# Bitlab-UMA/IMSAME

Measured on AMD Instinct MI355X. Metric: reads aligned/sec (node), 1M×150bp vs 50Mbp ref, 1/2/4/8 MI355X, higher is better.
Workload: dtype int16

## Files before the change

### imsame_amd/csrc/imsame_dev.hip

```cpp
#include <hip/hip_runtime.h>
#include <stdint.h>
#include <stdio.h>
#include <stdlib.h>
#include <string.h>
#include <math.h>
#include <limits.h>
#include <time.h>
#include <sched.h>
#include <vector>
#include <algorithm>
#include <thread>
#include <mutex>
#include <condition_variable>
#include "../../include/imsame_dev.h"

#include "tables.h"
#include "nw_kernel.hip"
#include "nw16_kernel.hip"
#include "nwl_kernel.hip"
#include "nwp_kernel.hip"
#include "seed_kernel.hip"
#include "round_policy.h"


// ... 255 lines not shown
    uint64_t tab_L = 0;
    uint32_t tab_ymax = 0, tab_xmax = 0;
    DBuf tb, bnd, paths, ck;
    DBuf slotbits;
    int np_part_cu = -1;
    DBuf np_tb, np_ck;
    imsame_ctx *np_owner = nullptr;
    uint64_t paths_cap_dev = 0, paths_n = 0;
    double paths_hint = 0;
    std::vector<uint32_t> paths_host;
    bool paths_on_host = false;
    DBuf rc_in, rc_out, rc_a, rc_b, rc_c;
    uint64_t ev_db_len = 0;
    bool use_wcap = false, use_wstart = false;
    DBuf wcap, wout, wstart;
    std::vector<imsame_ctx *> subs;
    bool is_sub = false, paths_split = false;
    std::vector<uint64_t> lane_paths;
    hipEvent_t origin = nullptr;
    hipEvent_t ev_w = nullptr;
    hipEvent_t ev_wd = nullptr;
    std::vector<std::pair<float, float>> nw_iv;
    struct TlEv { char kind; int round; uint32_t n; float a, b; };
    std::vector<TlEv> tl;
    int cur_round = 0;
    std::mutex iv_mu, persist_mu;
    int nlanes = 1;
    std::vector<uint32_t> part_paths;
    uint32_t stall_us[2] = {0, 0}, stall_n[2] = {0, 0};
};

static inline uint64_t hqs(const imsame_ctx *c, uint64_t r) { return c->hq[r - c->q_lo]; }
#define QB_READS 4096
static uint64_t range_ymax(const imsame_ctx *c, uint64_t a, uint64_t b) {
    uint64_t m = 0;
    auto len = [&](uint64_t r) { return hqs(c, r + 1) - hqs(c, r); };
    uint64_t blk = (a - c->q_lo + QB_READS - 1) / QB_READS, r = c->q_lo + blk * QB_READS;
    for (uint64_t x = a; x < std::min(b, r); ++x) m = std::max(m, len(x));
    for (; r + QB_READS <= b; r += QB_READS, ++blk) m = std::max<uint64_t>(m, c->hqb[blk]);
    for (uint64_t x = std::max(a, r); x < b; ++x) m = std::max(m, len(x));
    return m;
}
static inline const uint8_t *dev_q(const imsame_ctx *c) { return (const uint8_t *)((uintptr_t)c->q.p - c->q_base); }
static inline const uint32_t *dev_qw(const imsame_ctx *c) {
    return (const uint32_t *)((uintptr_t)c->qw.p - c->qw_base * sizeof(uint32_t));
}
static inline const uint64_t *dev_qs(const imsame_ctx *c) {
    return (const uint64_t *)((uintptr_t)c->q_start.p - c->q_lo * sizeof(uint64_t));
}
#define QPAD 64

enum { C_NCAND = 0, C_NCAND2, C_NNEXT, C_NCANDB, C_NCAND2B, C_NNEXT2, C_WORKB,
       C_WORK, C_WORK2, C_PATHS, C_FLAGS, C_ERR, C_HITS, C_CELLS, C_NACC, C_REDO,
       C_PROF, C_WIN = C_PROF + 12, C_FBK, C_SWORK, C_DBG = C_SWORK + 3, C_WASTE = C_DBG + 8,
       C_NSLOTS };

#define STALL_US_MAX 20000u
__global__ void __launch_bounds__(64) stall_kernel(uint32_t ticks) {
    const uint64_t t0 = wall_clock64();
    for (uint32_t i = 0; i < (1u << 20); ++i) {
        if (wall_clock64() - t0 >= ticks) break;
        __builtin_amdgcn_s_sleep(32);
    }
}
static void stall_parse(imsame_ctx *c) {
    c->stall_us[0] = c->stall_us[1] = 0;
    c->stall_n[0] = c->stall_n[1] = 0;
    const char *e = getenv("IMSAME_DEBUG_STALL");
    while (e && *e) {
        const int side = (*e == 'A' || *e == 'a') ? 0 : (*e == 'B' || *e == 'b') ? 1 : -1;
        if (side >= 0 && e[1] == ':') {
            const long us = strtol(e + 2, nullptr, 10);
            c->stall_us[side] = (uint32_t)std::max<long>(0, std::min<long>(us, (long)STALL_US_MAX));
        }
        e = strchr(e, ',');
        if (e) ++e;
    }
}
static int stall(imsame_ctx *c, hipStream_t s) {
    const int side = s == c->stream ? 0 : 1;
    if (!c->stall_us[side]) return 0;
    stall_kernel<<<1, 64, 0, s>>>(c->stall_us[side] * 100u);
    HIPCHK(hipGetLastError());
    __atomic_fetch_add(&c->stall_n[side], 1u, __ATOMIC_RELAXED);
    return 0;
}
#define STALL(c, s) do { if (int src_ = stall((c), (s))) return src_; } while (0)

static double now_ms() {
    struct timespec ts; clock_gettime(CLOCK_MONOTONIC, &ts);
    return ts.tv_sec * 1e3 + ts.tv_nsec * 1e-6;
}

extern "C" void imsame_params_default(imsame_params *p) {
    memset(p, 0, sizeof *p);
    p->min_e = 1 / powl(10, 20);
    p->min_coverage = 0.5; p->min_identity = 0.5;
    p->igap = -5; p->egap = -2;
    p->max_read_size = IMSAME_MAX_READ_SIZE;
    p->want_paths = 0;
}

extern "C" const char *imsame_strerror(int code) {
    switch (code) {
    case IMSAME_OK: return "ok";
    case IMSAME_E_HIP: return "HIP runtime error";
    case IMSAME_E_OOM: return "out of memory";
// ... 1509 lines not shown
                           (uint32_t *)(ctr + cls[k].work), c->db.as<uint8_t>(), c->db_start.as<uint64_t>(), qd, qsd,
                           pcap, &ms, k == 0 ? crow : nullptr);
            if (rc) return rc;
            rec_launch(st, pl, cls[k].n, ms);
            if ((rc = upd_launch(cls[k].cr, cls[k].cs, cls[k].n, cls[k].o, nxt, C_NNEXT, s))) return rc;
        }
        uint64_t nn = 0;
        HIPCHK(hipMemcpyAsync(&nn, ctr + C_NNEXT, 8, hipMemcpyDeviceToHost, s));
        LANE_SYNC(c, s);
        if (getenv("IMSAME_DEBUG_ROUNDS")) {
            std::vector<imsame_read_result> o(std::min<uint32_t>(n1, 6));
            std::vector<uint32_t> cr(o.size());
            if (!o.empty()) {
                HIPCHK(hipMemcpy(o.data(), c->cout.p, o.size() * 64, hipMemcpyDeviceToHost));
                HIPCHK(hipMemcpy(cr.data(), c->cread.p, o.size() * 4, hipMemcpyDeviceToHost));
            }
            uint64_t dg[8], nacc = 0;
            HIPCHK(hipMemcpy(dg, ctr + C_DBG, sizeof dg, hipMemcpyDeviceToHost));
            HIPCHK(hipMemcpy(&nacc, ctr + C_NACC, 8, hipMemcpyDeviceToHost));
            fprintf(stderr, "[round %llu] active=%u spec=%u budget=%u cand=%u+%u next=%llu acc_total=%llu "
                    "outcomes(err0 pause0 done0 err pause exh full)=%llu %llu %llu %llu %llu %llu %llu |",
                    (unsigned long long)st.rounds, nact, S.spec, S.budget, n1, n2, (unsigned long long)nn,
                    (unsigned long long)nacc, (unsigned long long)dg[0], (unsigned long long)dg[1],
                    (unsigned long long)dg[2], (unsigned long long)dg[3], (unsigned long long)dg[4],
                    (unsigned long long)dg[5], (unsigned long long)dg[6]);
            for (size_t k = 0; k < o.size(); ++k)
                fprintf(stderr, " r%u/s%llu st%u len%u id%u y%u", cr[k], (unsigned long long)o[k].db_seq, o[k].status,
                        o[k].length, o[k].identities, o[k].ylen);
            fprintf(stderr, "\n");
        }
        nact = (uint32_t)nn;
        std::swap(act, nxt);
    }
    uint64_t hc[C_NSLOTS];
    HIPCHK(hipMemcpyAsync(hc, ctr, C_NSLOTS * 8, hipMemcpyDeviceToHost, s));
    LANE_SYNC(c, s);
    const double t_d2h = now_ms();
    HIPCHK(hipMemcpyAsync(res, c->res.p, (uint64_t)n * 64, hipMemcpyDeviceToHost, s));
    LANE_SYNC(c, s);
    st.ms_d2h = now_ms() - t_d2h;
    st.n_hits = hc[C_HITS];
    st.seed_windows = hc[C_SWORK]; st.seed_entries = hc[C_SWORK + 1]; st.seed_ext_chunks = hc[C_SWORK + 2];
    st.nw_cells = hc[C_CELLS];
    st.n_accepted = hc[C_NACC];
    st.nw_redo = (uint32_t)hc[C_REDO];
    st.nw_win = (uint32_t)hc[C_WIN];
    st.nw_fallback = (uint32_t)hc[C_FBK];
    st.nw_spec_waste = hc[C_WASTE];
    if (getenv("IMSAME_NW_PROF")) {
        const double tot = (double)(hc[C_PROF] + hc[C_PROF + 1] + hc[C_PROF + 2] + hc[C_PROF + 3] + hc[C_PROF + 4]);
        const double ghz = hc[C_PROF + 5] ? tot / (double)hc[C_PROF + 5] * 0.1 : 0.0;
        fprintf(stderr, "[nwprof] setup %.3f sweep1 %.3f reduce %.3f sweep2 %.3f walk %.3f (fractions of %.4g wave-cycles) "
                "clock_ghz %.3f best_cells(weak: last_row last_col<=40 <=200 higher | predicted: in out) "
                "%llu %llu %llu %llu | %llu %llu\n", hc[C_PROF] / tot, hc[C_PROF + 1] / tot, hc[C_PROF + 2] / tot,
                hc[C_PROF + 3] / tot, hc[C_PROF + 4] / tot, tot, ghz, (unsigned long long)hc[C_PROF + 6],
                (unsigned long long)hc[C_PROF + 7], (unsigned long long)hc[C_PROF + 8], (unsigned long long)hc[C_PROF + 9],
                (unsigned long long)hc[C_PROF + 10], (unsigned long long)hc[C_PROF + 11]);
    }
    if ((c->stall_us[0] || c->stall_us[1]) && getenv("IMSAME_DEBUG_ROUNDS"))
        fprintf(stderr, "[stall] A=%u B=%u\n", c->stall_n[0], c->stall_n[1]);
    st.nw_launch_ms = st.nw_launches ? st.ms_nw / st.nw_launches : 0;
    st.nw_bytes = 2 * st.nw_cells;
    int ret = IMSAME_OK;
    if (hc[C_FLAGS] & 4) return IMSAME_E_HIP;
    if (hc[C_FLAGS] & 8) return IMSAME_E_ARG;
    if (hc[C_ERR] != ~0ull) {
        st.err_read = hc[C_ERR] >> 32; st.err_dbseq = hc[C_ERR] & 0xFFFFFFFFull;
        ret = IMSAME_E_READ_TOO_LONG;
    }
    if (p->want_paths) {
        uint64_t used = std::min<uint64_t>((uint32_t)hc[C_PATHS], pcap);
        if (hc[C_FLAGS] & 1) {
            rc = rewalk_lost(c, p, read_from, n, res, ymax, xcap, ycap, short_y, &used, &st);
            if (rc) return rc;
        }
        c->paths_n = used;
        c->paths_hint = std::min(64.0, (double)used / n);
        if (paths_used) *paths_used = used;
        if (used > paths_cap) { if (ret == IMSAME_OK) ret = IMSAME_E_PATHS; }
        else if (used) {
            HIPCHK(hipMemcpyAsync(paths, c->paths.p, used * 4, hipMemcpyDeviceToHost, s));
            HIPCHK(hipStreamSynchronize(s));
        }
    }
    st.ms_total = now_ms() - t_start;
    if (stats) *stats = st;
    return ret;
}

static void span_ms(const std::vector<std::pair<float, float>> &v, double *first, double *last) {
    *first = *last = 0;
    for (size_t k = 0; k < v.size(); ++k) {
        if (k == 0 || v[k].first < *first) *first = v[k].first;
        if (k == 0 || v[k].second > *last) *last = v[k].second;
    }
}

static double union_ms(std::vector<std::pair<float, float>> v) {
    std::sort(v.begin(), v.end());
    double tot = 0, a = 0, b = -1;
    for (const auto &x : v) {
        if (x.first > b) { if (b > a) tot += b - a; a = x.first; b = x.second; }
        else b = std::max<double>(b, x.second);
    }
    if (b > a) tot += b - a;
    return tot;
}

#define LANE_MIN 32768
#define LANE_READS 40000
// ... 496 lines not shown
```

### imsame_amd/csrc/nw16_kernel.hip

```cpp

#define NW16_K   10
#define NW16_K5  5
#define NW16_K3  3
#define NW16_K3_YMAX 150
#define NW16_BIG 16384
__host__ __device__ constexpr int nw16_ck(int K) { return K <= 3 ? 14 : K <= 5 ? 32 : 48; }
__host__ __device__ constexpr int nw16_nst(int K) { return 4 * K + 5; }
__host__ __device__ constexpr int nw16_nrec(int K) { return K <= 8 ? 2 : K <= 10 ? 3 : 2 * ((K + 7) / 8); }
#define NW16_K19 19
#define NW16_K19_OFF 2
#define NW16_K19_YLEN (8 * NW16_K19 - NW16_K19_OFF)
#define NW16_NOROW INT32_MIN
#define NW16_WIN_UP 32
#define NW16_WIN_DOWN 24
#define NW16_WIN_MAX 448
#define NW16_WIN_BOTTOM 40
#define NW16_BAND2 4

__host__ static inline bool nw16_fits(int64_t ig, int64_t eg, uint64_t xcap, uint64_t ymax, int K = NW16_K) {
    if (ig > 0 || eg > 0 || ymax > (uint64_t)NW_W / 2 || ymax == 0) return false;
    const uint64_t G = (ymax + K - 1) / K, ycols = G * K;
    const uint64_t aig = (uint64_t)(-ig), aeg = (uint64_t)(-eg);
    if (aig > 8191 || aeg > 8191) return false;
    const uint64_t R = 4 * ycols + aig + aeg * (xcap + 64 + ycols + 2) + 16;
    return R <= 8191;
}

WV_DEVICE uint32_t pk1(int v) { return (uint32_t)(uint16_t)v * 0x10001u; }
WV_DEVICE uint32_t pk2(int lo, int hi) { return (uint32_t)(uint16_t)lo | ((uint32_t)(uint16_t)hi << 16); }
WV_DEVICE int pk_half(uint32_t v, int h) { return (int)(int16_t)(h ? (v >> 16) : (v & 0xFFFFu)); }
#define NW16_H 0x80008000u
WV_DEVICE int pk_score(uint32_t v, int h) { return (int)(h ? (v >> 16) : (v & 0xFFFFu)) - 32768; }
WV_DEVICE uint32_t base_code(uint8_t b) { return (b >> 1) & 3u; }

#ifndef NW16_ROWTAB
#define NW16_ROWTAB 1
#endif
#define NW16_TBL_LO 0xFCFCFC04u
#define NW16_TBL_HI 0xFFFFFF00u
#if NW16_ROWTAB
#define NW16_XSH_A 3
#define NW16_XSH_B 5
#else
#define NW16_XSH_A 0
#define NW16_XSH_B 2
#endif
#define NW16_XM_A (3u << NW16_XSH_A)
#define NW16_XM_B (3u << NW16_XSH_B)
struct Nw16Row { uint32_t lo, hi; };
WV_DEVICE Nw16Row nw16_row(uint32_t xb) {
#if NW16_ROWTAB
    return {8u << (xb & 31u), 8u << ((xb >> 2) & 0x18u)};
#else
    return {wv_perm(xb >> 2, xb & 3u, 0x04040000u), 0u};
#endif
}
WV_DEVICE uint32_t nw16_ycol(uint32_t ya, uint32_t yb) {
#if NW16_ROWTAB
    return ya | (0x0Cu << 8) | ((yb + 4u) << 16) | (0x0Cu << 24);
#else
    return ya | ((ya | 4u) << 8) | (yb << 16) | ((yb | 4u) << 24);
#endif
}
WV_DEVICE uint32_t nw16_sc(const Nw16Row &r, uint32_t ycol) {
#if NW16_ROWTAB
    return wv_perm(r.hi, r.lo, ycol);
#else
    return wv_perm(NW16_TBL_HI, NW16_TBL_LO, r.lo ^ ycol);
#endif
// ... 74 lines not shown
};

__host__ __device__ static inline size_t nw16_wave_lds(int GPW, int xstride) {
    return (size_t)GPW * xstride + 64 * 8 * 4;
}

template <int K, bool LAST, bool TWO, int OFF = 0>
__device__ __forceinline__ void nw16_wave(const NwLaunch &P, uint8_t *wsm, const int lane, const uint32_t slot) {
    constexpr int NST = nw16_nst(K), NREC = nw16_nrec(K), CK = nw16_ck(K);
    constexpr uint32_t RECB = 64u * 4u * NREC;
    const int G = P.G, GPW = P.GPW;
    const int g = lane / G, gl = lane - g * G;
    const bool in_group = g < GPW;
    const int gg = in_group ? g : 0;
    int *red = (int *)(wsm + (size_t)GPW * P.xstride);
    uint32_t *tbw = P.tb + (uint64_t)slot * P.tb_wave_dw;
    uint32_t *ckw = TWO ? P.ck + (uint64_t)slot * P.ck_wave_dw + lane : nullptr;
    const int ig = P.igap, eg = P.egap;

    unsigned long long ph[5] = {0, 0, 0, 0, 0}, tq = P.prof ? wv_clock() : 0, rt0 = P.prof ? wv_realtime() : 0;
    auto mark = [&](const int k) {
        if (P.prof) { const unsigned long long n = wv_clock(); ph[k] += n - tq; tq = n; }
    };
    for (uint32_t ntask = 0;; ++ntask) {
        if (P.slot_bits && ntask) break;
        uint32_t base = 0;
        if (lane == 0) base = wv_atomic_add(P.counter, (uint32_t)(2 * GPW));
        base = wv_first(base);
        if (base >= P.n_cand) break;
        bool valid[2];
        uint32_t cidx[2], sid[2] = {0, 0};
        int xl[2] = {0, 0}, yl[2] = {0, 0}, prow[2] = {NW16_NOROW, NW16_NOROW};
        const uint8_t *Yp[2] = {P.q, P.q}, *Xg[2] = {P.db, P.db};
        for (int h = 0; h < 2; ++h) {
            cidx[h] = base + 2 * g + h;
            valid[h] = in_group && cidx[h] < P.n_cand;
        }
        for (int h = 0; h < 2; ++h) {
            const uint32_t w = valid[h] ? cidx[h] : cidx[0];
            if (valid[0]) {
                const uint32_t c = P.perm ? P.perm[w] : w;
                cidx[h] = c;
                if (P.cand_row) prow[h] = P.cand_row[c];
                const uint32_t rd = P.cand_read[c];
                sid[h] = P.cand_sid[c];
                const uint64_t xo = P.db_start[sid[h]];
                xl[h] = (int)(P.db_start[sid[h] + 1] - xo);
                Xg[h] = P.db + xo;
                const uint64_t yo = P.q_start[rd];
                Yp[h] = P.q + yo; yl[h] = (int)(P.q_start[rd + 1] - yo);
            }
        }
        const int xlp = max(xl[0], xl[1]);
        uint8_t *X8 = wsm + (size_t)(valid[0] ? g : 0) * P.xstride;
        if (valid[0]) {
            const int nch = (xlp + 15) >> 4;
            for (int c = gl; c < nch; c += G) {
                const int k0 = c << 4;
                uint32_t w[2][4];
                for (int h = 0; h < 2; ++h) {
                    if (k0 + 16 <= xl[h]) {
                        __builtin_memcpy(w[h], Xg[h] + k0, 16);
                    } else {
#pragma unroll
                        for (int q = 0; q < 4; ++q) {
                            uint32_t v = 0;
#pragma unroll
                            for (int b = 0; b < 4; ++b) v |= (uint32_t)Xg[h][min(k0 + 4 * q + b, xl[h] - 1)] << (8 * b);
                            w[h][q] = v;
                        }
                    }
                }
                uint32_t o[4];
#pragma unroll
                for (int q = 0; q < 4; ++q)
                    o[q] = (((w[0][q] >> 1) << NW16_XSH_A) & (NW16_XM_A * 0x01010101u)) |
                           (((w[1][q] >> 1) << NW16_XSH_B) & (NW16_XM_B * 0x01010101u));
                __builtin_memcpy(X8 + k0, o, 16);
            }
        }
        wv_lds_sync();

        int xmax = valid[0] ? xlp : 0, xmin = valid[0] ? min(xl[0], xl[1]) : INT_MAX;
        for (int o = 32; o > 0; o >>= 1) {
            xmax = max(xmax, wv_shfl_xor(xmax, o));
            xmin = min(xmin, wv_shfl_xor(xmin, o));
        }
        xmax = (int)wv_first((uint32_t)xmax); xmin = (int)wv_first((uint32_t)xmin);
        int tw0 = INT_MAX - 2, tw1 = INT_MAX - 2;
        if (TWO && P.cand_row) {
            int lo = INT_MAX, hi = INT_MIN, none = 0;
            for (int h = 0; h < 2; ++h) {
                if (!valid[h]) continue;
                if (prow[h] == NW16_NOROW) {
                    if (P.win_bottom < 0) { none = 1; continue; }
                    lo = min(lo, xl[h] - 1 - P.win_bottom);
                    hi = max(hi, xl[h] - 1);
                    continue;
                }
                lo = min(lo, prow[h] - P.win_up);
                hi = max(hi, prow[h] + yl[h] - 1 + P.win_down);
            }
            for (int o = 32; o > 0; o >>= 1) {
                lo = min(lo, wv_shfl_xor(lo, o));
                hi = max(hi, wv_shfl_xor(hi, o));
                none = max(none, wv_shfl_xor(none, o));
            }
            if (!none && lo <= hi) {
                int a = max(lo, 1), b = min(hi, xmax) + G;
                a -= (a & 1) ^ 1; b += (b & 1) ^ 1;
                if (b > a && b - a <= NW16_WIN_MAX) { tw0 = a; tw1 = b; }
            }
            tw0 = (int)wv_first((uint32_t)tw0); tw1 = (int)wv_first((uint32_t)tw1);
        }
        const int tb0 = TWO ? tw0 : 0;

        const int j0 = gl * K - OFF;
        const bool leadc0 = gl == 0;
        const int xcl = max(xlp - 1, 0);
        const uint32_t NBIG = pk1(-NW16_BIG) ^ NW16_H, EGN = pk1(-eg), IGEN = pk1(-(ig + eg));
        uint32_t yreg[K], lastm[K];
        bool ownC[2], lact[2];
        for (int h = 0; h < 2; ++h) {
            ownC[h] = valid[0] && yl[h] >= 2 && yl[h] - 1 >= j0 && yl[h] - 1 < j0 + K;
            lact[h] = valid[0] && j0 < yl[h];
        }
#pragma unroll
        for (int s = 0; s < K; ++s) {
            const int j = j0 + s;
            const uint32_t ya = (valid[0] && j >= 0 && j < yl[0]) ? base_code(Yp[0][j]) : 0u;
            const uint32_t yb = (valid[0] && j >= 0 && j < yl[1]) ? base_code(Yp[1][j]) : 0u;
            yreg[s] = nw16_ycol(ya, yb);
            lastm[s] = ((ownC[0] && yl[0] - 1 - j0 == s) ? 0x0000FFFFu : 0u) |
                       ((ownC[1] && yl[1] - 1 - j0 == s) ? 0xFFFF0000u : 0u);
        }
        uint32_t xrow = valid[0] ? X8[0] : 0u;
        const Nw16Row xr0 = nw16_row(xrow);
        uint32_t yprev = nw16_ycol(0u, 0u);
        if (valid[0] && j0 > 0) {
            const uint32_t ya = base_code(Yp[0][min(j0 - 1, yl[0] - 1)]), yb = base_code(Yp[1][min(j0 - 1, yl[1] - 1)]);
            yprev = nw16_ycol(ya, yb);
        }
        const uint32_t t0prev = nw16_sc_biased(nw16_sc(xr0, yprev));
        uint32_t A[K], B[K], dI[K], mcS[K], u0[K];
#pragma unroll
        for (int s = 0; s < K; ++s) {
            A[s] = nw16_sc_biased(nw16_sc(xr0, yreg[s]));
            B[s] = A[s];
        }
#pragma unroll
        for (int s = 0; s < K; ++s) {
            dI[s] = ((s == 0) ? t0prev : A[s - 1]) - IGEN;
            mcS[s] = dI[s];
            u0[s] = dI[s];
            if (j0 + s == 1) mcS[s] = pk1(NW16_BIG) ^ NW16_H;
        }
        uint32_t I1 = t0prev, I2 = t0prev;
        uint32_t outT = A[K - 1], outMS = 0, outL = 0;
        const int tend = xmax - 1 + G;
        xrow = valid[0] ? X8[min(max(1 - gl, 0), xcl)] : 0u;
        uint32_t bestC = pk1(-NW16_BIG) ^ NW16_H, bestCi = 0, ipk = pk1(1 - gl);
        int bestR[2] = {INT_MIN, INT_MIN}, bestRj[2] = {0, 0};
        const uint32_t limp = pk2(xl[0] - 2, xl[1] - 2);
        uint8_t *tb3 = (uint8_t *)tbw;

        auto step = [&](const bool PRE, const bool CAREFUL, const bool TB, const int t, uint32_t (&cur)[K],
                        const uint32_t (&own)[K], uint32_t &in0, const uint32_t in1) {
            const uint32_t sN = (uint32_t)wv_shr1((int)outT), mS = (uint32_t)wv_shr1((int)outMS),
                           mL0 = (uint32_t)wv_shr1((int)outL);
            const int i = t - gl;
            const Nw16Row xr = nw16_row(xrow);
            xrow = CAREFUL ? X8[min(max(i + 1, 0), xcl)] : X8[i + 1];
            const bool pre = PRE && i < 1;
            const bool row1 = CAREFUL && i <= 1;
            uint32_t mfS = mS, l0 = mL0;
            TbWords<K> tw = {};
#pragma unroll
            for (int s = 0; s < K; ++s) {
                const uint32_t d0 = (s == 0) ? in1 : own[s - 1];
                const uint32_t tl = (s == 0) ? sN : cur[s - 1];
                const uint32_t sc = nw16_sc(xr, yreg[s]);
                const uint32_t up = row1 ? NBIG : u0[s];
                const uint32_t lu = pk_maxu(l0, up);
                uint32_t v = nw16_add_sc(pk_maxu(d0, lu), sc);
                if (s == OFF) v = leadc0 ? nw16_sc_biased(sc) : v;
                cur[s] = pre ? own[s] : v;
                const uint32_t P2 = TB ? wv_perm(pk_sub(l0, up), pk_sub(d0, lu), 0x0B0A0908u) : 0u;
                const uint32_t mU = pk_neg_mask(pk_sub(mcS[s], dI[s]));
                const uint32_t u0n = wv_bfi(mU, dI[s], u0[s]) - EGN;
                u0[s] = row1 ? u0[s] : u0n;
                mcS[s] = wv_bfi(mU, dI[s], mcS[s]);
                const uint32_t mnL = pk_neg_mask(pk_sub(tl, mfS));
                dI[s] = d0 - IGEN;
                l0 = wv_bfi(mnL, l0 - EGN, dI[s]);
                mfS = wv_bfi(mnL, mfS, d0);
                if (s == OFF) { mfS = leadc0 ? NBIG : mfS; l0 = leadc0 ? NBIG : l0; }
                if (TB) tw.add(s, P2, mU, mnL);
            }
            if (TB) tw.store((uint32_t *)(tb3 + ((uint32_t)(t - tb0) * RECB + (uint32_t)lane * (4u * NREC))));
            uint32_t vl = cur[LAST ? K - 1 : 0];
            if (!LAST)
#pragma unroll
                for (int s = 1; s < K; ++s) vl = wv_bfi(lastm[s], cur[s], vl);
            uint32_t km = pk_neg_mask(pk_sub(vl, bestC));
            if (CAREFUL) {
                km |= pk_neg_mask(pk_sub(limp, ipk)) | pk_neg_mask(pk_sub(ipk, pk1(1)));
                if (i >= 1 && (i == xl[0] - 1 || i == xl[1] - 1)) {
                    for (int h = 0; h < 2; ++h) {
                        if (!lact[h] || i != xl[h] - 1) continue;
#pragma unroll
                        for (int s = 0; s < K; ++s) {
                            const int j = j0 + s, val = pk_score(cur[s], h);
                            if (j >= 1 && j < yl[h] && val >= bestR[h]) { bestR[h] = val; bestRj[h] = j; }
                        }
                    }
                }
            }
            bestC = wv_bfi(km, bestC, vl);
            bestCi = wv_bfi(km, bestCi, ipk);
            ipk = pk_add(ipk, 0x10001u);
            in0 = pre ? in1 : sN;
            outT = cur[K - 1]; outMS = mfS; outL = l0;
        };
        constexpr bool TB1 = !TWO;
        auto save = [&](const int m) {
            uint32_t *p = ckw + (uint32_t)m * (NST * 64u);
#pragma unroll
            for (int s = 0; s < K; ++s) {
                p[s * 64] = A[s]; p[(K + s) * 64] = B[s];
                p[(2 * K + s) * 64] = mcS[s]; p[(3 * K + s) * 64] = u0[s];
            }
            p[4 * K * 64] = I1; p[(4 * K + 1) * 64] = I2;
            p[(4 * K + 2) * 64] = outT; p[(4 * K + 3) * 64] = outMS; p[(4 * K + 4) * 64] = outL;
        };
        int nextck = 1 + CK, mck = 1;
        auto ck = [&](const int t) { if (TWO && t == nextck) { save(mck); ++mck; nextck += CK; } };
        if (TWO) save(0);
        mark(0);
        auto inwin = [&](const int tt) { return TWO && tt >= tw0 && tt < tw1; };
        int t = 1;
        for (; t + 1 < tend && t <= G + 1; t += 2) {
            ck(t);
            if (inwin(t)) {
                step(true, true, true, t, A, B, I2, I1);
                step(true, true, true, t + 1, B, A, I1, I2);
            } else {
                step(true, true, TB1, t, A, B, I2, I1);
                step(true, true, TB1, t + 1, B, A, I1, I2);
            }
        }
        auto fast = [&](const bool TBW, const int tlim) {
            for (; t + 1 <= tlim; t += 2) {
                ck(t);
                step(false, false, TBW, t, A, B, I2, I1);
                step(false, false, TBW, t + 1, B, A, I1, I2);
            }
        };
        fast(TB1, min(xmin - 2, tw0 - 1));
        if (TWO) {
            fast(true, min(xmin - 2, tw1 - 1));
            fast(false, xmin - 2);
        }
        for (; t + 1 < tend; t += 2) {
            ck(t);
            if (inwin(t)) {
                step(false, true, true, t, A, B, I2, I1);
                step(false, true, true, t + 1, B, A, I1, I2);
            } else {
                step(false, true, TB1, t, A, B, I2, I1);
                step(false, true, TB1, t + 1, B, A, I1, I2);
            }
        }
        if (t < tend) {
            if (inwin(t)) step(true, true, true, t, A, B, I2, I1);
            else          step(true, true, TB1, t, A, B, I2, I1);
        }
        wv_mem_sync();
        mark(1);

        for (int h = 0; h < 2; ++h) {
            red[lane * 8 + 4 * h + 0] = bestR[h];
            red[lane * 8 + 4 * h + 1] = bestRj[h];
            red[lane * 8 + 4 * h + 2] = ownC[h] ? pk_score(bestC, h) : INT_MIN;
            red[lane * 8 + 4 * h + 3] = pk_half(bestCi, h);
        }
        wv_lds_sync();
        int bscore[2], bx[2], by[2];
        for (int h = 0; h < 2; ++h) {
            int bR = INT_MIN, bRj = 0, bC = INT_MIN, bCi = 0;
            if (in_group)
                for (int k = 0; k < G; ++k) {
                    const int *e = red + (g * G + k) * 8 + 4 * h;
                    if (e[0] > bR || (e[0] == bR && e[1] > bRj)) { bR = e[0]; bRj = e[1]; }
                    if (e[2] > bC || (e[2] == bC && e[3] > bCi)) { bC = e[2]; bCi = e[3]; }
                }
            if (bR >= bC) { bscore[h] = bR; bx[h] = xl[h] - 1; by[h] = bRj; }
            else          { bscore[h] = bC; bx[h] = bCi; by[h] = yl[h] - 1; }
        }
        wv_lds_sync();
        if (P.prof && in_group && gl == 0)
            for (int h = 0; h < 2; ++h) {
                if (!valid[h]) continue;
                int b;
                if (prow[h] == NW16_NOROW) {
                    const int up = xl[h] - 1 - bx[h];
                    b = up == 0 ? 6 : up <= 40 ? 7 : up <= 200 ? 8 : 9;
                } else {
                    b = (bx[h] >= prow[h] - P.win_up && bx[h] <= prow[h] + yl[h] - 1 + P.win_down) ? 10 : 11;
                }
                wv_atomic_add64(P.prof + b, 1ull);
            }
        mark(2);
        if (!TWO) {
            for (int h = 0; h < 2; ++h) {
                const TbAcc16<K, OFF> acc16 = {tbw, X8, Yp[h], gg, G, h, 0};
                nw_finish(P, acc16, xl[h], yl[h], valid[h], gg, gl, G, bscore[h], bx[h], by[h], cidx[h], sid[h]);
            }
            wv_lds_sync();
            mark(4);
            continue;
        }

        bool todo[2] = {valid[0], valid[1]};
        if (tw1 > tw0) {
            bool cov[2];
            for (int h = 0; h < 2; ++h) cov[h] = todo[h] && bx[h] + G <= tw1;
            if (wv_any(cov[0] || cov[1])) {
                for (int h = 0; h < 2; ++h) {
                    TbAcc16<K, OFF> acc16 = {tbw, X8, Yp[h], gg, G, h, tw0};
                    acc16.t1 = tw1;
                    const bool lost = nw_finish(P, acc16, xl[h], yl[h], cov[h], gg, gl, G, bscore[h], bx[h], by[h],
                                                cidx[h], sid[h]);
                    if (cov[h]) todo[h] = lost;
                    if (cov[h] && !lost && gl == 0 && in_group && P.win) wv_atomic_add(P.win, 1u);
                }
                wv_mem_sync();
            }
            mark(4);
        }
        int t0h[2] = {1, 1};
        auto step2 = [&](const bool MASK, const int tau, uint32_t (&cur)[K], const uint32_t (&own)[K],
                         uint32_t &in0, const uint32_t in1) {
            const uint32_t sN = (uint32_t)wv_shr1((int)outT), mS = (uint32_t)wv_shr1((int)outMS),
                           mL0 = (uint32_t)wv_shr1((int)outL);
            const int iA = t0h[0] + tau - gl, iB = t0h[1] + tau - gl;
            const Nw16Row xr = nw16_row(xrow);
            xrow = (X8[min(max(iA + 1, 0), xcl)] & NW16_XM_A) | (X8[min(max(iB + 1, 0), xcl)] & NW16_XM_B);
            const uint32_t pm = !MASK ? 0u : (iA < 1 ? 0x0000FFFFu : 0u) | (iB < 1 ? 0xFFFF0000u : 0u);
            const uint32_t r1 = !MASK ? 0u : (iA <= 1 ? 0x0000FFFFu : 0u) | (iB <= 1 ? 0xFFFF0000u : 0u);
            uint32_t mfS = mS, l0 = mL0;
            TbWords<K> tw = {};
#pragma unroll
            for (int s = 0; s < K; ++s) {
                const uint32_t d0 = (s == 0) ? in1 : own[s - 1];
                const uint32_t tl = (s == 0) ? sN : cur[s - 1];
                const uint32_t sc = nw16_sc(xr, yreg[s]);
                const uint32_t up = MASK ? wv_bfi(r1, NBIG, u0[s]) : u0[s];
                const uint32_t lu = pk_maxu(l0, up);
                uint32_t v = nw16_add_sc(pk_maxu(d0, lu), sc);
                if (s == OFF) v = leadc0 ? nw16_sc_biased(sc) : v;
                cur[s] = MASK ? wv_bfi(pm, own[s], v) : v;
                const uint32_t P2 = wv_perm(pk_sub(l0, up), pk_sub(d0, lu), 0x0B0A0908u);
                const uint32_t mU = pk_neg_mask(pk_sub(mcS[s], dI[s]));
                const uint32_t u0n = wv_bfi(mU, dI[s], u0[s]) - EGN;
                u0[s] = MASK ? wv_bfi(r1, u0[s], u0n) : u0n;
                mcS[s] = wv_bfi(mU, dI[s], mcS[s]);
                const uint32_t mnL = pk_neg_mask(pk_sub(tl, mfS));
                dI[s] = d0 - IGEN;
                l0 = wv_bfi(mnL, l0 - EGN, dI[s]);
                mfS = wv_bfi(mnL, mfS, d0);
                if (s == OFF) { mfS = leadc0 ? NBIG : mfS; l0 = leadc0 ? NBIG : l0; }
                tw.add(s, P2, mU, mnL);
            }
            tw.store((uint32_t *)(tb3 + ((uint32_t)tau * RECB + (uint32_t)lane * (4u * NREC))));
            in0 = MASK ? wv_bfi(pm, in1, sN) : sN;
            outT = cur[K - 1]; outMS = mfS; outL = l0;
        };
        for (int att = wv_any(todo[0] || todo[1]) ? 0 : 3; att < 3; ++att) {
            int n2 = 0;
            for (int h = 0; h < 2; ++h) {
                const int lo = bx[h] - (att == 0 ? P.band_w : NW16_BAND2 * P.band_w) - 1;
                t0h[h] = (att < 2 && lo >= 0) ? 1 + CK * (lo / CK) : 1;
                if (todo[h]) n2 = max(n2, bx[h] + G - t0h[h]);
            }
            for (int o = 32; o > 0; o >>= 1) n2 = max(n2, wv_shfl_xor(n2, o));
            {
                const uint32_t *pa = ckw + (uint32_t)((t0h[0] - 1) / CK) * (NST * 64u);
                const uint32_t *pb = ckw + (uint32_t)((t0h[1] - 1) / CK) * (NST * 64u);
                auto ld = [&](const int r) { return wv_bfi(0x0000FFFFu, pa[r * 64], pb[r * 64]); };
#pragma unroll
                for (int s = 0; s < K; ++s) {
                    A[s] = ld(s); B[s] = ld(K + s);
                    mcS[s] = ld(2 * K + s); u0[s] = ld(3 * K + s);
                }
                I1 = ld(4 * K); I2 = ld(4 * K + 1);
                outT = ld(4 * K + 2); outMS = ld(4 * K + 3); outL = ld(4 * K + 4);
#pragma unroll
                for (int s = 0; s < K; ++s) dI[s] = (s ? A[s - 1] : I2) - IGEN;
                xrow = (X8[min(max(t0h[0] - gl, 0), xcl)] & NW16_XM_A) | (X8[min(max(t0h[1] - gl, 0), xcl)] & NW16_XM_B);
            }
            int tmin = min(t0h[0], t0h[1]);
            for (int o = 32; o > 0; o >>= 1) tmin = min(tmin, wv_shfl_xor(tmin, o));
            const int tau_m = G + 1 - tmin;
            int tau = 0;
            for (; tau + 1 < n2 && tau < tau_m; tau += 2) {
                step2(true, tau, A, B, I2, I1);
                step2(true, tau + 1, B, A, I1, I2);
            }
            for (; tau + 1 < n2; tau += 2) {
                step2(false, tau, A, B, I2, I1);
                step2(false, tau + 1, B, A, I1, I2);
            }
            if (tau < n2) step2(true, tau, A, B, I2, I1);
            wv_mem_sync();
            mark(3);
            for (int h = 0; h < 2; ++h) {
                const TbAcc16<K, OFF> acc16 = {tbw, X8, Yp[h], gg, G, h, t0h[h]};
                todo[h] = nw_finish(P, acc16, xl[h], yl[h], todo[h], gg, gl, G, bscore[h], bx[h], by[h], cidx[h],
                                    sid[h]);
            }
            mark(4);
            if (!wv_any(todo[0] || todo[1])) break;
            if (lane == 0 && P.redo) wv_atomic_add(P.redo, 1u);
            wv_mem_sync();
        }
        wv_lds_sync();
    }
    if (P.prof && lane == 0) {
        for (int k = 0; k < 5; ++k) wv_atomic_add64(P.prof + k, ph[k]);
        wv_atomic_add64(P.prof + 5, wv_realtime() - rt0);
    }
}

__host__ static inline NwShape nw16_shape(uint32_t ymax, uint32_t xcap, int K = NW16_K) {
    NwShape s;
    s.k = K;
    s.G = (int)((ymax + K - 1) / K);
    if (s.G < 1) s.G = 1;
    s.GPW = 64 / s.G; s.nstr = 1;
    s.xcap = xcap < 2 ? 2 : (int)xcap;
    s.xstride = (s.xcap + 15) & ~15;
    while (s.GPW > 1 && (size_t)s.GPW * s.xstride > 16384) s.GPW--;
    s.steps = s.xcap + s.G;
    return s;
}
__host__ static inline bool nw16_k19_ok(uint32_t ylen_uni, uint32_t ymax, uint32_t xcap, const imsame_params *p) {
    const char *e = getenv("IMSAME_NW_K19"), *k = getenv("IMSAME_NW_K");
    if ((e && !atoi(e)) || (k && atoi(k) != NW16_K19)) return false;
    if (ylen_uni != NW16_K19_YLEN || ymax != NW16_K19_YLEN) return false;
    if (!nw16_fits(p->igap, p->egap, xcap, ymax, NW16_K19)) return false;
    const NwShape s = nw16_shape(ymax, xcap, NW16_K19);
    return s.G * s.GPW == 64;
}
__host__ static inline uint64_t nw16_tb_words(const NwShape &s) { return (uint64_t)s.steps * 64 * nw16_nrec(s.k); }
__host__ static inline uint64_t nw16_ck_words(const NwShape &s) {
    return (uint64_t)((s.steps + nw16_ck(s.k) - 1) / nw16_ck(s.k) + 1) * nw16_nst(s.k) * 64;
}

#ifndef IMSAME_WAVE_EMU
__device__ __forceinline__ uint32_t nw_xcc_id() {
    uint32_t v;
    asm volatile("s_getreg_b32 %0, hwreg(HW_REG_XCC_ID, 0, 4)" : "=s"(v));
    return v;
}
__device__ uint32_t nw_slot_claim(const NwLaunch &P, const int lane) {
    const uint32_t part = nw_xcc_id() & 7u, nw = P.slot_words;
    uint32_t *bits = P.slot_bits + part * nw;
    uint32_t got = ~0u;
    if (lane == 0) {
        uint32_t w = blockIdx.x % nw;
        for (uint32_t it = 0; it < (1u << 22) && got == ~0u; ++it) {
            uint32_t v = __hip_atomic_load(bits + w, __ATOMIC_RELAXED, __HIP_MEMORY_SCOPE_AGENT);
            while (v != 0xFFFFFFFFu) {
                const uint32_t b = (uint32_t)__builtin_ctz(~v);
                const uint32_t old = __hip_atomic_fetch_or(bits + w, 1u << b, __ATOMIC_RELAXED, __HIP_MEMORY_SCOPE_AGENT);
                if (!(old & (1u << b))) { got = (part * nw + w) * 32u + b; break; }
                v = old | (1u << b);
            }
            if (got == ~0u && ++w == nw) { w = 0; __builtin_amdgcn_s_sleep(4); }
        }
    }
    got = __builtin_amdgcn_readfirstlane(wv_shfl((int)got, 0));
    __builtin_amdgcn_fence(__ATOMIC_ACQUIRE, "agent");
    return got;
}
__device__ __forceinline__ void nw_slot_release(const NwLaunch &P, const int lane, const uint32_t slot) {
    __builtin_amdgcn_s_waitcnt(0);
    if (lane == 0)
        __hip_atomic_fetch_and(P.slot_bits + (slot >> 5), ~(1u << (slot & 31u)), __ATOMIC_RELAXED,
                               __HIP_MEMORY_SCOPE_AGENT);
}

__global__ void xcc_probe_kernel(uint32_t *out) {
    if (threadIdx.x == 0) out[blockIdx.x] = nw_xcc_id();
// ... 37 lines not shown
```

### imsame_amd/csrc/wave_ops.h

```cpp
#pragma once

#ifndef IMSAME_WAVE_EMU
#include <hip/hip_runtime.h>

#define WV_DEVICE __device__ __forceinline__

WV_DEVICE int wv_shr1(int v) { return __builtin_amdgcn_mov_dpp(v, 0x138, 0xf, 0xf, true); }
WV_DEVICE int wv_shl1(int v) { return __builtin_amdgcn_mov_dpp(v, 0x130, 0xf, 0xf, true); }
WV_DEVICE int wv_shr1_fill(int v, int fill) { return __builtin_amdgcn_update_dpp(fill, v, 0x138, 0xf, 0xf, false); }
WV_DEVICE int wv_shl1_fill(int v, int fill) { return __builtin_amdgcn_update_dpp(fill, v, 0x130, 0xf, 0xf, false); }
WV_DEVICE int wv_max3(int a, int b, int c) {
    int r;
    asm("v_max3_i32 %0, %1, %2, %3" : "=v"(r) : "v"(a), "v"(b), "v"(c));
    return r;
}
WV_DEVICE unsigned long long wv_ballot(bool p) { return __ballot(p); }
WV_DEVICE bool wv_any(bool p) { return __any(p); }
WV_DEVICE int wv_shfl(int v, int src) { return __shfl(v, src); }
WV_DEVICE int wv_shfl_xor(int v, int m) { return __shfl_xor(v, m); }
WV_DEVICE uint32_t wv_first(uint32_t v) { return __builtin_amdgcn_readfirstlane(v); }
WV_DEVICE int wv_readlane(int v, int l) { return __builtin_amdgcn_readlane(v, l); }
WV_DEVICE uint32_t wv_atomic_add(uint32_t *p, uint32_t v) { return atomicAdd(p, v); }
WV_DEVICE void wv_atomic_or(uint32_t *p, uint32_t v) { atomicOr(p, v); }
WV_DEVICE void wv_atomic_min64(unsigned long long *p, unsigned long long v) { atomicMin(p, v); }
WV_DEVICE void wv_atomic_add64(unsigned long long *p, unsigned long long v) { atomicAdd(p, v); }
WV_DEVICE unsigned long long wv_clock() { return (unsigned long long)clock64(); }
WV_DEVICE unsigned long long wv_realtime() { return (unsigned long long)__builtin_amdgcn_s_memrealtime(); }
WV_DEVICE void wv_lds_sync() {
    __builtin_amdgcn_fence(__ATOMIC_RELEASE, "wavefront");
    __builtin_amdgcn_wave_barrier();
    __builtin_amdgcn_fence(__ATOMIC_ACQUIRE, "wavefront");
}
WV_DEVICE void wv_mem_sync() {
    __builtin_amdgcn_s_waitcnt(0);
    __threadfence_block();
}

typedef short wv_s2 __attribute__((ext_vector_type(2)));
WV_DEVICE wv_s2 pk_v(uint32_t a) { return __builtin_bit_cast(wv_s2, a); }
WV_DEVICE uint32_t pk_u(wv_s2 a) { return __builtin_bit_cast(uint32_t, a); }
WV_DEVICE uint32_t pk_add(uint32_t a, uint32_t b) { return pk_u(pk_v(a) + pk_v(b)); }
WV_DEVICE uint32_t pk_sub(uint32_t a, uint32_t b) { return pk_u(pk_v(a) - pk_v(b)); }
WV_DEVICE uint32_t pk_max(uint32_t a, uint32_t b) { return pk_u(__builtin_elementwise_max(pk_v(a), pk_v(b))); }
typedef unsigned short wv_u2 __attribute__((ext_vector_type(2)));
WV_DEVICE uint32_t pk_maxu(uint32_t a, uint32_t b) {
    return __builtin_bit_cast(uint32_t, __builtin_elementwise_max(__builtin_bit_cast(wv_u2, a), __builtin_bit_cast(wv_u2, b)));
}
WV_DEVICE uint32_t pk_minu(uint32_t a, uint32_t b) {
    return __builtin_bit_cast(uint32_t, __builtin_elementwise_min(__builtin_bit_cast(wv_u2, a), __builtin_bit_cast(wv_u2, b)));
}
WV_DEVICE uint32_t pk_neg_mask(uint32_t a) {
    uint32_t r;
    asm("v_pk_ashrrev_i16 %0, 15, %1 op_sel_hi:[0,1]" : "=v"(r) : "v"(a));
    return r;
}
WV_DEVICE uint32_t wv_and_or(uint32_t m, uint32_t c, uint32_t w) {
    uint32_t r;
    asm("v_bitop3_b32 %0, %1, %2, %3 bitop3:0xea" : "=v"(r) : "v"(m), "v"(c), "v"(w));
    return r;
}
WV_DEVICE uint32_t wv_bfi(uint32_t m, uint32_t a, uint32_t b) {
    uint32_t r;
    asm("v_bitop3_b32 %0, %1, %2, %3 bitop3:0xca" : "=v"(r) : "v"(m), "v"(a), "v"(b));
    return r;
}
WV_DEVICE uint32_t wv_perm(uint32_t hi, uint32_t lo, uint32_t sel) { return __builtin_amdgcn_perm(hi, lo, sel); }
WV_DEVICE uint32_t wv_alignbit(uint32_t hi, uint32_t lo, uint32_t s) { return __builtin_amdgcn_alignbit(hi, lo, s); }
WV_DEVICE uint32_t wv_bitrev(uint32_t v) { return __builtin_bitreverse32(v); }
WV_DEVICE uint32_t wv_shift_in(uint32_t w, bool c) {
    uint32_t r;
    unsigned long long co;
    asm("v_addc_co_u32_e64 %0, %1, %2, %2, %3" : "=v"(r), "=s"(co) : "v"(w), "s"(__builtin_amdgcn_ballot_w64(c)));
    return r;
}

#else
#include <stdint.h>
#include <string.h>
#include <climits>
#include <algorithm>
#include <atomic>

#define WV_DEVICE inline
#define __host__
#define __device__
#define __global__
#define __forceinline__ inline
#define __launch_bounds__(...)
#define __restrict__
using std::max;
using std::min;
struct uint2 { uint32_t x, y; };
inline uint2 make_uint2(uint32_t x, uint32_t y) { return uint2{x, y}; }

namespace wvemu {
struct Wave;
extern thread_local Wave *t_wave;
extern thread_local int t_lane;
void sync();
extern thread_local uint64_t *t_xch;
}

inline int wv_lane() { return wvemu::t_lane; }
inline int __mul24(int a, int b) { return a * b; }
inline int wv_max3(int a, int b, int c) { return std::max(a, std::max(b, c)); }
inline int wv_shr1(int v) {
    wvemu::t_xch[wvemu::t_lane] = (uint64_t)(uint32_t)v;
    wvemu::sync();
    int r = wvemu::t_lane ? (int)(uint32_t)wvemu::t_xch[wvemu::t_lane - 1] : 0;
    wvemu::sync();
    return r;
}
inline int wv_shl1(int v) {
    wvemu::t_xch[wvemu::t_lane] = (uint64_t)(uint32_t)v;
    wvemu::sync();
    int r = wvemu::t_lane < 63 ? (int)(uint32_t)wvemu::t_xch[wvemu::t_lane + 1] : 0;
    wvemu::sync();
    return r;
}
inline int wv_shr1_fill(int v, int fill) {
    wvemu::t_xch[wvemu::t_lane] = (uint64_t)(uint32_t)v;
    wvemu::sync();
    int r = wvemu::t_lane ? (int)(uint32_t)wvemu::t_xch[wvemu::t_lane - 1] : fill;
    wvemu::sync();
    return r;
}
inline int wv_shl1_fill(int v, int fill) {
    wvemu::t_xch[wvemu::t_lane] = (uint64_t)(uint32_t)v;
    wvemu::sync();
    int r = wvemu::t_lane < 63 ? (int)(uint32_t)wvemu::t_xch[wvemu::t_lane + 1] : fill;
    wvemu::sync();
    return r;
}
inline unsigned long long wv_ballot(bool p) {
    wvemu::t_xch[wvemu::t_lane] = p;
    wvemu::sync();
    unsigned long long m = 0;
    for (int l = 0; l < 64; ++l) m |= (unsigned long long)(wvemu::t_xch[l] & 1) << l;
    wvemu::sync();
    return m;
}
inline bool wv_any(bool p) { return wv_ballot(p) != 0; }
inline int wv_shfl(int v, int src) {
    wvemu::t_xch[wvemu::t_lane] = (uint64_t)(uint32_t)v;
    wvemu::sync();
    int r = (int)(uint32_t)wvemu::t_xch[((src % 64) + 64) % 64];
    wvemu::sync();
    return r;
}
inline int wv_shfl_xor(int v, int m) { return wv_shfl(v, wvemu::t_lane ^ m); }
inline uint32_t wv_first(uint32_t v) { return (uint32_t)wv_shfl((int)v, 0); }
inline int wv_readlane(int v, int l) { return wv_shfl(v, l); }
inline uint32_t wv_atomic_add(uint32_t *p, uint32_t v) {
    return __atomic_fetch_add(p, v, __ATOMIC_SEQ_CST);
}
inline void wv_atomic_or(uint32_t *p, uint32_t v) { __atomic_fetch_or(p, v, __ATOMIC_SEQ_CST); }
inline void wv_atomic_min64(unsigned long long *p, unsigned long long v) {
    unsigned long long cur = __atomic_load_n(p, __ATOMIC_SEQ_CST);
    while (v < cur && !__atomic_compare_exchange_n(p, &cur, v, false, __ATOMIC_SEQ_CST, __ATOMIC_SEQ_CST)) {}
}
inline void wv_atomic_add64(unsigned long long *p, unsigned long long v) { __atomic_fetch_add(p, v, __ATOMIC_SEQ_CST); }
inline unsigned long long wv_clock() { return 0; }
inline unsigned long long wv_realtime() { return 0; }
inline void wv_lds_sync() { wvemu::sync(); }
inline void wv_mem_sync() { wvemu::sync(); }

inline uint32_t pk_map(uint32_t a, uint32_t b, int (*f)(int, int)) {
    const int lo = f((int16_t)(a & 0xFFFF), (int16_t)(b & 0xFFFF)), hi = f((int16_t)(a >> 16), (int16_t)(b >> 16));
    return ((uint32_t)(uint16_t)lo) | ((uint32_t)(uint16_t)hi << 16);
}
inline uint32_t pk_add(uint32_t a, uint32_t b) { return pk_map(a, b, [](int x, int y) { return x + y; }); }
inline uint32_t pk_sub(uint32_t a, uint32_t b) { return pk_map(a, b, [](int x, int y) { return x - y; }); }
inline uint32_t pk_max(uint32_t a, uint32_t b) { return pk_map(a, b, [](int x, int y) { return x > y ? x : y; }); }
inline uint32_t pk_maxu(uint32_t a, uint32_t b) {
    const uint32_t lo = std::max(a & 0xFFFFu, b & 0xFFFFu), hi = std::max(a >> 16, b >> 16);
    return lo | (hi << 16);
}
inline uint32_t pk_minu(uint32_t a, uint32_t b) {
    const uint32_t lo = std::min(a & 0xFFFFu, b & 0xFFFFu), hi = std::min(a >> 16, b >> 16);
    return lo | (hi << 16);
}
inline uint32_t pk_neg_mask(uint32_t a) { return pk_map(a, 0, [](int x, int) { return x < 0 ? -1 : 0; }); }
inline uint32_t wv_shift_in(uint32_t w, bool c) { return (w << 1) | (c ? 1u : 0u); }
inline uint32_t wv_and_or(uint32_t m, uint32_t c, uint32_t w) { return (m & c) | w; }
inline uint32_t wv_bfi(uint32_t m, uint32_t a, uint32_t b) { return (m & a) | (~m & b); }
inline uint32_t wv_alignbit(uint32_t hi, uint32_t lo, uint32_t s) {
    return (uint32_t)((((uint64_t)hi << 32) | lo) >> (s & 31));
}
inline uint32_t wv_bitrev(uint32_t v) {
    uint32_t r = 0;
    for (int k = 0; k < 32; ++k) r |= ((v >> k) & 1u) << (31 - k);
    return r;
}
inline uint32_t wv_perm(uint32_t hi, uint32_t lo, uint32_t sel) {
    const uint64_t v = ((uint64_t)hi << 32) | lo;
    uint32_t r = 0;
    for (int k = 0; k < 4; ++k) {
        const uint32_t s = (sel >> (8 * k)) & 0xFF;
        uint32_t b;
        if (s < 8) b = (uint32_t)(v >> (8 * s)) & 0xFF;
        else if (s == 12) b = 0;
        else if (s > 12) b = 0xFF;
        else b = ((v >> (s == 8 ? 15 : s == 9 ? 31 : s == 10 ? 47 : 63)) & 1) ? 0xFF : 0;
        r |= b << (8 * k);
    }
    return r;
}
#endif
```

Baseline: 10.35 million.

## Restructure NW16 sweep into head/tail phases with padded X rows and separate row-best tracking

```diff
diff --git a/imsame_amd/csrc/imsame_dev.hip b/imsame_amd/csrc/imsame_dev.hip
--- a/imsame_amd/csrc/imsame_dev.hip
+++ b/imsame_amd/csrc/imsame_dev.hip
@@ -331,7 +331,7 @@
 
 enum { C_NCAND = 0, C_NCAND2, C_NNEXT, C_NCANDB, C_NCAND2B, C_NNEXT2, C_WORKB,
        C_WORK, C_WORK2, C_PATHS, C_FLAGS, C_ERR, C_HITS, C_CELLS, C_NACC, C_REDO,
-       C_PROF, C_WIN = C_PROF + 12, C_FBK, C_SWORK, C_DBG = C_SWORK + 3, C_WASTE = C_DBG + 8,
+       C_PROF, C_WIN = C_PROF + 14, C_FBK, C_SWORK, C_DBG = C_SWORK + 3, C_WASTE = C_DBG + 8,
        C_NSLOTS };
 
 #define STALL_US_MAX 20000u
@@ -1947,10 +1947,11 @@
         const double ghz = hc[C_PROF + 5] ? tot / (double)hc[C_PROF + 5] * 0.1 : 0.0;
         fprintf(stderr, "[nwprof] setup %.3f sweep1 %.3f reduce %.3f sweep2 %.3f walk %.3f (fractions of %.4g wave-cycles) "
                 "clock_ghz %.3f best_cells(weak: last_row last_col<=40 <=200 higher | predicted: in out) "
-                "%llu %llu %llu %llu | %llu %llu\n", hc[C_PROF] / tot, hc[C_PROF + 1] / tot, hc[C_PROF + 2] / tot,
+                "%llu %llu %llu %llu | %llu %llu weak_window_waves(all skipped_second_sweep) %llu %llu\n", hc[C_PROF] / tot, hc[C_PROF + 1] / tot, hc[C_PROF + 2] / tot,
                 hc[C_PROF + 3] / tot, hc[C_PROF + 4] / tot, tot, ghz, (unsigned long long)hc[C_PROF + 6],
                 (unsigned long long)hc[C_PROF + 7], (unsigned long long)hc[C_PROF + 8], (unsigned long long)hc[C_PROF + 9],
-                (unsigned long long)hc[C_PROF + 10], (unsigned long long)hc[C_PROF + 11]);
+                (unsigned long long)hc[C_PROF + 10], (unsigned long long)hc[C_PROF + 11],
+                (unsigned long long)hc[C_PROF + 12], (unsigned long long)hc[C_PROF + 13]);
     }
     if ((c->stall_us[0] || c->stall_us[1]) && getenv("IMSAME_DEBUG_ROUNDS"))
         fprintf(stderr, "[stall] A=%u B=%u\n", c->stall_n[0], c->stall_n[1]);
diff --git a/imsame_amd/csrc/nw16_kernel.hip b/imsame_amd/csrc/nw16_kernel.hip
--- a/imsame_amd/csrc/nw16_kernel.hip
+++ b/imsame_amd/csrc/nw16_kernel.hip
@@ -14,7 +14,7 @@
 #define NW16_WIN_UP 32
 #define NW16_WIN_DOWN 24
 #define NW16_WIN_MAX 448
-#define NW16_WIN_BOTTOM 40
+#define NW16_WIN_BOTTOM (-1)
 #define NW16_BAND2 4
 
 __host__ static inline bool nw16_fits(int64_t ig, int64_t eg, uint64_t xcap, uint64_t ymax, int K = NW16_K) {
@@ -195,15 +195,25 @@
             }
         }
         const int xlp = max(xl[0], xl[1]);
+        int xmax = valid[0] ? xlp : 0, xmin = valid[0] ? min(xl[0], xl[1]) : INT_MAX;
+        for (int o = 32; o > 0; o >>= 1) {
+            xmax = max(xmax, wv_shfl_xor(xmax, o));
+            xmin = min(xmin, wv_shfl_xor(xmin, o));
+        }
+        xmax = (int)wv_first((uint32_t)xmax); xmin = (int)wv_first((uint32_t)xmin);
         uint8_t *X8 = wsm + (size_t)(valid[0] ? g : 0) * P.xstride;
         if (valid[0]) {
-            const int nch = (xlp + 15) >> 4;
+            const int nch = (xmax + G + 1 + 15) >> 4;
             for (int c = gl; c < nch; c += G) {
                 const int k0 = c << 4;
                 uint32_t w[2][4];
                 for (int h = 0; h < 2; ++h) {
                     if (k0 + 16 <= xl[h]) {
                         __builtin_memcpy(w[h], Xg[h] + k0, 16);
+                    } else if (k0 >= xl[h]) {
+                        const uint32_t v = (uint32_t)Xg[h][xl[h] - 1] * 0x01010101u;
+#pragma unroll
+                        for (int q = 0; q < 4; ++q) w[h][q] = v;
                     } else {
 #pragma unroll
                         for (int q = 0; q < 4; ++q) {
@@ -224,12 +234,6 @@
         }
         wv_lds_sync();
 
-        int xmax = valid[0] ? xlp : 0, xmin = valid[0] ? min(xl[0], xl[1]) : INT_MAX;
-        for (int o = 32; o > 0; o >>= 1) {
-            xmax = max(xmax, wv_shfl_xor(xmax, o));
-            xmin = min(xmin, wv_shfl_xor(xmin, o));
-        }
-        xmax = (int)wv_first((uint32_t)xmax); xmin = (int)wv_first((uint32_t)xmin);
         int tw0 = INT_MAX - 2, tw1 = INT_MAX - 2;
         if (TWO && P.cand_row) {
             int lo = INT_MAX, hi = INT_MIN, none = 0;
@@ -302,20 +306,21 @@
         uint32_t outT = A[K - 1], outMS = 0, outL = 0;
         const int tend = xmax - 1 + G;
         xrow = valid[0] ? X8[min(max(1 - gl, 0), xcl)] : 0u;
-        uint32_t bestC = pk1(-NW16_BIG) ^ NW16_H, bestCi = 0, ipk = pk1(1 - gl);
-        int bestR[2] = {INT_MIN, INT_MIN}, bestRj[2] = {0, 0};
+        uint32_t bestC = pk1(-NW16_BIG) ^ NW16_H, bestCt = pk1(gl);
+        const uint32_t glpk = pk1(gl);
+        for (int h = 0; h < 2; ++h) { red[lane * 8 + 4 * h + 0] = INT_MIN; red[lane * 8 + 4 * h + 1] = 0; }
         const uint32_t limp = pk2(xl[0] - 2, xl[1] - 2);
         uint8_t *tb3 = (uint8_t *)tbw;
 
-        auto step = [&](const bool PRE, const bool CAREFUL, const bool TB, const int t, uint32_t (&cur)[K],
-                        const uint32_t (&own)[K], uint32_t &in0, const uint32_t in1) {
+        auto step = [&](const bool HEAD, const bool TAIL, const bool TB, const int t, uint32_t (&cur)[K],
+                        const uint32_t (&own)[K], uint32_t &in0, const uint32_t in1) WV_LAMBDA_INLINE {
             const uint32_t sN = (uint32_t)wv_shr1((int)outT), mS = (uint32_t)wv_shr1((int)outMS),
                            mL0 = (uint32_t)wv_shr1((int)outL);
             const int i = t - gl;
             const Nw16Row xr = nw16_row(xrow);
-            xrow = CAREFUL ? X8[min(max(i + 1, 0), xcl)] : X8[i + 1];
-            const bool pre = PRE && i < 1;
-            const bool row1 = CAREFUL && i <= 1;
+            xrow = HEAD ? X8[max(i + 1, 0)] : X8[i + 1];
+            const bool pre = HEAD && i < 1;
+            const bool row1 = HEAD && i <= 1;
             uint32_t mfS = mS, l0 = mL0;
             TbWords<K> tw = {};
 #pragma unroll
@@ -346,24 +351,32 @@
 #pragma unroll
                 for (int s = 1; s < K; ++s) vl = wv_bfi(lastm[s], cur[s], vl);
             uint32_t km = pk_neg_mask(pk_sub(vl, bestC));
-            if (CAREFUL) {
-                km |= pk_neg_mask(pk_sub(limp, ipk)) | pk_neg_mask(pk_sub(ipk, pk1(1)));
-                if (i >= 1 && (i == xl[0] - 1 || i == xl[1] - 1)) {
-                    for (int h = 0; h < 2; ++h) {
-                        if (!lact[h] || i != xl[h] - 1) continue;
-#pragma unroll
-                        for (int s = 0; s < K; ++s) {
-                            const int j = j0 + s, val = pk_score(cur[s], h);
-                            if (j >= 1 && j < yl[h] && val >= bestR[h]) { bestR[h] = val; bestRj[h] = j; }
-                        }
-                    }
-                }
+            const uint32_t tpk = (uint32_t)t * 0x10001u;
+            if (HEAD || TAIL) {
+                const uint32_t ipk = pk_sub(tpk, glpk);
+                if (TAIL) km |= pk_neg_mask(pk_sub(limp, ipk));
+                if (HEAD) km |= pk_neg_mask(pk_sub(ipk, pk1(1)));
             }
             bestC = wv_bfi(km, bestC, vl);
-            bestCi = wv_bfi(km, bestCi, ipk);
-            ipk = pk_add(ipk, 0x10001u);
+            bestCt = wv_bfi_u(km, bestCt, tpk);
             in0 = pre ? in1 : sN;
             outT = cur[K - 1]; outMS = mfS; outL = l0;
+        };
+        auto rowbest = [&](const int t, const uint32_t (&cur)[K]) WV_LAMBDA_INLINE {
+            const int i = t - gl;
+            const bool hit = i >= 1 && (i == xl[0] - 1 || i == xl[1] - 1);
+            if (!wv_any(hit)) return;
+            if (hit)
+                for (int h = 0; h < 2; ++h) {
+                    if (!lact[h] || i != xl[h] - 1) continue;
+                    int bR = INT_MIN, bRj = 0;
+#pragma unroll
+                    for (int s = 0; s < K; ++s) {
+                        const int j = j0 + s, val = pk_score(cur[s], h);
+                        if (j >= 1 && j < yl[h] && val >= bR) { bR = val; bRj = j; }
+                    }
+                    red[lane * 8 + 4 * h + 0] = bR; red[lane * 8 + 4 * h + 1] = bRj;
+                }
         };
         constexpr bool TB1 = !TWO;
         auto save = [&](const int m) {
@@ -380,52 +393,41 @@
         auto ck = [&](const int t) { if (TWO && t == nextck) { save(mck); ++mck; nextck += CK; } };
         if (TWO) save(0);
         mark(0);
-        auto inwin = [&](const int tt) { return TWO && tt >= tw0 && tt < tw1; };
         int t = 1;
-        for (; t + 1 < tend && t <= G + 1; t += 2) {
-            ck(t);
-            if (inwin(t)) {
-                step(true, true, true, t, A, B, I2, I1);
-                step(true, true, true, t + 1, B, A, I1, I2);
-            } else {
-                step(true, true, TB1, t, A, B, I2, I1);
-                step(true, true, TB1, t + 1, B, A, I1, I2);
-            }
-        }
-        auto fast = [&](const bool TBW, const int tlim) {
-            for (; t + 1 <= tlim; t += 2) {
+        auto pairs = [&](const bool HEAD, const bool TAIL, const bool TBW, const int tlim) WV_LAMBDA_INLINE {
+            t = (int)wv_first((uint32_t)t);
+            const int tl = (int)wv_first((uint32_t)tlim);
+            for (; t + 1 <= tl; t += 2) {
                 ck(t);
-                step(false, false, TBW, t, A, B, I2, I1);
-                step(false, false, TBW, t + 1, B, A, I1, I2);
+                step(HEAD, TAIL, TBW, t, A, B, I2, I1);
+                if (TAIL) rowbest(t, A);
+                step(HEAD, TAIL, TBW, t + 1, B, A, I1, I2);
+                if (TAIL) rowbest(t + 1, B);
             }
         };
-        fast(TB1, min(xmin - 2, tw0 - 1));
-        if (TWO) {
-            fast(true, min(xmin - 2, tw1 - 1));
-            fast(false, xmin - 2);
-        }
-        for (; t + 1 < tend; t += 2) {
-            ck(t);
-            if (inwin(t)) {
-                step(false, true, true, t, A, B, I2, I1);
-                step(false, true, true, t + 1, B, A, I1, I2);
-            } else {
-                step(false, true, TB1, t, A, B, I2, I1);
-                step(false, true, TB1, t + 1, B, A, I1, I2);
-            }
-        }
+        auto sweep = [&](const bool HEAD, const bool TAIL, const int tlim) WV_LAMBDA_INLINE {
+            pairs(HEAD, TAIL, TB1, min(tlim, tw0 - 1));
+            if (TWO) {
+                pairs(HEAD, TAIL, true, min(tlim, tw1 - 1));
+                pairs(HEAD, TAIL, false, tlim);
+            }
+        };
+        const int tpair = tend - 1, thead = min(tpair, G + 2);
+        sweep(true, false, min(thead, xmin - 2));
+        sweep(true, true, thead);
+        sweep(false, false, xmin - 2);
+        sweep(false, true, tpair);
         if (t < tend) {
-            if (inwin(t)) step(true, true, true, t, A, B, I2, I1);
-            else          step(true, true, TB1, t, A, B, I2, I1);
+            if (TWO && t >= tw0 && t < tw1) step(true, true, true, t, A, B, I2, I1);
+            else                            step(true, true, TB1, t, A, B, I2, I1);
+            rowbest(t, A);
         }
         wv_mem_sync();
         mark(1);
 
         for (int h = 0; h < 2; ++h) {
-            red[lane * 8 + 4 * h + 0] = bestR[h];
-            red[lane * 8 + 4 * h + 1] = bestRj[h];
             red[lane * 8 + 4 * h + 2] = ownC[h] ? pk_score(bestC, h) : INT_MIN;
-            red[lane * 8 + 4 * h + 3] = pk_half(bestCi, h);
+            red[lane * 8 + 4 * h + 3] = pk_half(bestCt, h) - gl;
         }
         wv_lds_sync();
         int bscore[2], bx[2], by[2];
@@ -478,6 +480,14 @@
                     if (cov[h] && !lost && gl == 0 && in_group && P.win) wv_atomic_add(P.win, 1u);
                 }
                 wv_mem_sync();
+            }
+            if (P.prof) {
+                const bool pred = wv_any((valid[0] && prow[0] != NW16_NOROW) || (valid[1] && prow[1] != NW16_NOROW));
+                const bool left = wv_any(todo[0] || todo[1]);
+                if (!pred && lane == 0) {
+                    wv_atomic_add64(P.prof + 12, 1ull);
+                    if (!left) wv_atomic_add64(P.prof + 13, 1ull);
+                }
             }
             mark(4);
         }
@@ -582,7 +592,7 @@
     if (s.G < 1) s.G = 1;
     s.GPW = 64 / s.G; s.nstr = 1;
     s.xcap = xcap < 2 ? 2 : (int)xcap;
-    s.xstride = (s.xcap + 15) & ~15;
+    s.xstride = (s.xcap + s.G + 1 + 15) & ~15;
     while (s.GPW > 1 && (size_t)s.GPW * s.xstride > 16384) s.GPW--;
     s.steps = s.xcap + s.G;
     return s;
diff --git a/imsame_amd/csrc/wave_ops.h b/imsame_amd/csrc/wave_ops.h
--- a/imsame_amd/csrc/wave_ops.h
+++ b/imsame_amd/csrc/wave_ops.h
@@ -4,6 +4,7 @@
 #include <hip/hip_runtime.h>
 
 #define WV_DEVICE __device__ __forceinline__
+#define WV_LAMBDA_INLINE __attribute__((always_inline))
 
 WV_DEVICE int wv_shr1(int v) { return __builtin_amdgcn_mov_dpp(v, 0x138, 0xf, 0xf, true); }
 WV_DEVICE int wv_shl1(int v) { return __builtin_amdgcn_mov_dpp(v, 0x130, 0xf, 0xf, true); }
@@ -64,6 +65,11 @@
     asm("v_bitop3_b32 %0, %1, %2, %3 bitop3:0xca" : "=v"(r) : "v"(m), "v"(a), "v"(b));
     return r;
 }
+WV_DEVICE uint32_t wv_bfi_u(uint32_t m, uint32_t a, uint32_t b) {
+    uint32_t r;
+    asm("v_bitop3_b32 %0, %1, %2, %3 bitop3:0xca" : "=v"(r) : "v"(m), "v"(a), "s"(b));
+    return r;
+}
 WV_DEVICE uint32_t wv_perm(uint32_t hi, uint32_t lo, uint32_t sel) { return __builtin_amdgcn_perm(hi, lo, sel); }
 WV_DEVICE uint32_t wv_alignbit(uint32_t hi, uint32_t lo, uint32_t s) { return __builtin_amdgcn_alignbit(hi, lo, s); }
 WV_DEVICE uint32_t wv_bitrev(uint32_t v) { return __builtin_bitreverse32(v); }
@@ -82,6 +88,7 @@
 #include <atomic>
 
 #define WV_DEVICE inline
+#define WV_LAMBDA_INLINE
 #define __host__
 #define __device__
 #define __global__
@@ -184,6 +191,7 @@
 inline uint32_t wv_shift_in(uint32_t w, bool c) { return (w << 1) | (c ? 1u : 0u); }
 inline uint32_t wv_and_or(uint32_t m, uint32_t c, uint32_t w) { return (m & c) | w; }
 inline uint32_t wv_bfi(uint32_t m, uint32_t a, uint32_t b) { return (m & a) | (~m & b); }
+inline uint32_t wv_bfi_u(uint32_t m, uint32_t a, uint32_t b) { return wv_bfi(m, a, b); }
 inline uint32_t wv_alignbit(uint32_t hi, uint32_t lo, uint32_t s) {
     return (uint32_t)((((uint64_t)hi << 32) | lo) >> (s & 31));
 }
```

Result: faster. 10.49 million, median of 6 (+1.4%).
